# Project-SEA-Stack/HydroChrono

Measured on AMD Instinct MI355X. Metric: hydro-force evals/sec (all bodies), higher is better.
Workload: dtype f64

## Files before the change

hydrochrono_amd/capi.py:

```python
import ctypes as C
import os

_PKG = os.path.dirname(os.path.abspath(__file__))
LIB_PATH = os.path.join(_PKG, "lib", "libhydrochrono_amd.so")
TUNING_LIB_PATH = os.path.join(_PKG, "lib", "libhydrochrono_amd_tuning.so")

HC_OK, HC_ERR_RUNTIME, HC_ERR_OUT_OF_RANGE, HC_ERR_INVALID, HC_ERR_DEVICE, HC_ERR_UNSUPPORTED = range(6)

c_double_p = C.POINTER(C.c_double)
c_int_p = C.POINTER(C.c_int)


class IrregularWaveParams(C.Structure):
    _fields_ = [("num_bodies", C.c_int), ("simulation_dt", C.c_double), ("simulation_duration", C.c_double),
                ("ramp_duration", C.c_double), ("wave_height", C.c_double), ("wave_period", C.c_double),
                ("frequency_min", C.c_double), ("frequency_max", C.c_double), ("nfrequencies", C.c_double),
                ("peak_enhancement_factor", C.c_double), ("is_normalized", C.c_int), ("seed", C.c_int)]


class TaperedDirectOptions(C.Structure):
    _fields_ = [("smoothing", C.c_int), ("window_length", C.c_int), ("rirf_end_time", C.c_double),
                ("taper_start_percent", C.c_double), ("taper_end_percent", C.c_double),
                ("taper_final_amplitude", C.c_double), ("export_plot_csv", C.c_int)]

# ... 15 lines not shown
                ("hydrostatics_calls", C.c_int), ("radiation_calls", C.c_int), ("waves_calls", C.c_int),
                ("conv_kernel_seconds", C.c_double), ("conv_kernel_launches", C.c_longlong),
                ("conv_kernel_bytes", C.c_double), ("block_kernel_seconds", C.c_double),
                ("block_kernel_launches", C.c_longlong), ("block_kernel_bytes", C.c_double),
                ("block_kernel_bytes_once", C.c_double),
                ("step_kernel_seconds", C.c_double), ("step_kernel_launches", C.c_longlong),
                ("scatter_kernel_seconds", C.c_double), ("scatter_kernel_launches", C.c_longlong),
                ("direct_dispatches", C.c_longlong), ("hip_launches", C.c_longlong), ("history_rewinds", C.c_longlong),
                ("mini_pass_seconds", C.c_double), ("mini_pass_launches", C.c_longlong), ("queue_parkings", C.c_longlong),
                ("ahead_pass_slices", C.c_longlong), ("ahead_blocks", C.c_longlong),
                ("pass_lane_launches", C.c_longlong),
                ("multi_doorbell_offset_last", C.c_double), ("multi_doorbell_offset_sum", C.c_double), ("multi_calls", C.c_longlong),
                ("slot_state_steps", C.c_longlong), ("wide_fused_steps", C.c_longlong),
                ("schedule_blocks_ahead", C.c_longlong), ("schedule_blocks_at_start", C.c_longlong), ("ring_grows_for_pass", C.c_longlong),
                ("hot_steps", C.c_longlong), ("tail_launches", C.c_longlong), ("tail_seconds", C.c_double),
                ("tail_bytes", C.c_double), ("tail_blocks", C.c_longlong)]


class InitStats(C.Structure):
    _fields_ = [("h5_read_seconds", C.c_double), ("h5_read_bytes", C.c_double), ("rirf_h2d_seconds", C.c_double), ("rirf_h2d_bytes", C.c_double),
                ("rirf_relayout_seconds", C.c_double), ("rirf_relayout_bytes", C.c_double), ("finalize_seconds", C.c_double),
                ("direct_setup_seconds", C.c_double), ("wave_resample_seconds", C.c_double), ("wave_spectrum_seconds", C.c_double),
                ("wave_eta_seconds", C.c_double), ("wave_eta_samples", C.c_longlong), ("wave_eta_components", C.c_longlong),
                ("wave_eta_mode", C.c_int), ("pad_", C.c_int), ("wave_upload_seconds", C.c_double), ("wave_upload_bytes", C.c_double),
                ("wave_total_seconds", C.c_double), ("taper_seconds", C.c_double), ("taper_bytes", C.c_double),
                ("synth_seconds", C.c_double), ("synth_bytes", C.c_double)]


SIGNATURES = {
    "hc_version": (C.c_char_p, []),
    "hc_device_count": (C.c_int, []),
# ... 179 lines not shown
```

hydrochrono_amd/csrc/hc_context.hpp:

```cpp
#pragma once
#include <hip/hip_runtime.h>

#include <chrono>
#include <deque>
#include <stdexcept>
#include <string>
#include <vector>

#include "../../include/hydrochrono_amd.h"
#include "hc_direct.hpp"
#include "hc_kernels.hpp"
#include "hc_plan.hpp"

namespace hc {

struct Error : std::runtime_error {
    int status;
    Error(int st, const std::string& what) : std::runtime_error(what), status(st) {}
};

#define HC_HIP(expr)                                                                                          \
    do {                                                                                                      \
        hipError_t _e = (expr);                                                                               \
        if (_e != hipSuccess)                                                                                 \
// ... 256 lines not shown
    int mt_mini = 2;
    int mt_narrow = 2;
    int mt_block = 4, mt_block_design = 6;
    int num_cus  = 256;
    int lookahead = 0;
    hc::Plan plan;
    unsigned long long plan_serial = 0;
    int pass_ahead = 0, pass_slices = 8, pe_cur = 0;
    bool ahead_now = false;
    int gap_seen = 0, gap_long = 0, gap_long_lo = 0;
    double gap_threshold = 4e-6;
    double gap_hint = -1.0;
    std::chrono::steady_clock::time_point t_multi_end{};
    bool have_t_multi_end = false;
    hc::AheadPass ahead;
    int radiation_tail = 1;
    struct SpectralTail {
        bool khat_ok = false;
        bool active = false;
        int k = 0, Q = 0;
        int cur = 0;
        unsigned far_cur = 0, far_next = 0;
        unsigned long long serial = 0;
        double t0 = 0.0, dt = 0.0;
    } spec;
    hc::DeviceBuffer<double> d_khat, d_tail_xw, d_tail_yfar, d_tail_out, d_tail_tw;
    hc::DirectKernel dk_tail_fwd, dk_tail_gemv, dk_tail_inv;
    hc::DeviceBuffer<double> d_partials_far;
    hc::DeviceBuffer<double> d_partials_next;
    bool pass_concurrent = true;
    int pass_lane = 0, pass_free_cus = 4;

    hc::DeviceBuffer<double> d_state, d_hs, d_rad, d_waves, d_total;
    hc::DeviceBuffer<double> d_scratch;
    hc::DeviceBuffer<int> d_err;
    hc::PinnedBuffer<double> h_state, h_out, h_am;
    hc::BarBuffer<double> bar_state;
    hc::BarBuffer<double> bar_am;
    hc::PinnedBuffer<unsigned long long> h_tag_am;
    int am_lane = 0;
    hc::BarBuffer<double> bar_selftest;
    hc::PinnedBuffer<unsigned long long> h_tag_selftest;
// ... 31 lines not shown
```

hydrochrono_amd/csrc/hc_internal.hpp:

```cpp
#pragma once
#include <dlfcn.h>
#include <fcntl.h>
#include <unistd.h>
#include <xmmintrin.h>

#include <algorithm>
#include <chrono>
#include <cmath>
#include <cstdint>
#include <cstdio>
#include <cstdlib>
#include <cstring>
#include <fstream>
#include <limits>
#include <memory>
#include <string>
#include <vector>

#include "hc_context.hpp"
#include "hc_history.hpp"
#include "hc_host_math.hpp"

namespace hc {
void eta_synthesis_fft(const std::vector<double>& t, const std::vector<double>& amp, const std::vector<double>& omega,
// ... 108 lines not shown
    hc::Panel kex;
    hc::EtaTable ex;
};
StepViews make_views(const hc_ctx* c);
struct PassSetup {
    hc::BlockArgs b;
    bool exc_block = false;
    double rad_once = 0.0, exc_once = 0.0, bytes_steps = 0.0;
};
PassSetup make_pass(hc_ctx* c, bool with_exc, bool next_block, bool head_only = false);
void issue_pass_chunks(hc_ctx* c, const PassSetup& ps, int first, int last, bool with_items, hipStream_t stream, bool direct, int lane = 0);
void issue_pass_reduce(hc_ctx* c, const PassSetup& ps, double* P, double* E, hipStream_t stream, bool direct, int lane = 0, const double* tail = nullptr,
                       int tail_j0 = 0);
void launch_pass(hc_ctx* c, hipStream_t stream, bool with_exc, bool direct = false, bool spec_goes_on = false);
void spec_drop(hc_ctx* c, bool k_changed);
void spec_build_khat(hc_ctx* c);
void launch_mini_pass(hc_ctx* c, int i0, hipStream_t stream, bool direct, int next_kw = 0, int lane = 0);
void ahead_drop(hc_ctx* c);
void ahead_issue_slice(hc_ctx* c, hipStream_t stream, bool direct);
void ahead_begin(hc_ctx* c, hipStream_t stream, bool with_exc, bool direct);
bool ahead_expected(const hc_ctx* c, unsigned long long ended_serial);
bool ahead_adoptable(const hc_ctx* c, unsigned long long ended_serial);
bool pass_lane_ready(hc_ctx* c);
void pass_lane_drain(hc_ctx* c);

}
}
```

hydrochrono_amd/csrc/hc_kernels.hip:

```cpp
#include "hc_kernels.hpp"

#include <algorithm>
#include <cstdint>
#include <cstdlib>

namespace hc {

static constexpr int kConvThreads = 256;
static constexpr int kWave        = 64;

typedef double dvec2 __attribute__((ext_vector_type(2)));
typedef double dvec2u __attribute__((ext_vector_type(2), aligned(8)));
typedef double dvec4 __attribute__((ext_vector_type(4)));

__host__ __device__ inline size_t panel_offset(int ngp, int row, int f) {
    const int rt = row >> 4, ri = row & 15, gp = f >> 3, j = (f >> 2) & 1, kk = f & 3;
    return ((static_cast<size_t>(rt) * ngp + gp) * 64 + (kk * 16 + ri)) * 2 + j;
}

__global__ void __launch_bounds__(256) relayout_rirf_kernel(const double* __restrict__ Kb, double* __restrict__ K, int ngp, int D, int S,
                                                             int row0, double scale) {
    const size_t F   = (size_t)S * D;
    const size_t gid = (size_t)blockIdx.x * blockDim.x + threadIdx.x;
    if (gid >= 6 * F) return;
// ... 1820 lines not shown
    NearLaunch l;
    a.n_slices = near_slices_for(a.D);
    const int groups = (a.D + 7) / 8 + 1;
    a.gps_per_slice = (((groups + a.n_slices - 1) / a.n_slices) + 3) & ~3;
    l.grid = a.K.ntiles * a.n_slices;
    l.smem = (size_t)max(1, a.n_near) * 8 * a.gps_per_slice * sizeof(double);
    return l;
}

void launch_near_split(const NearArgs& a0, hipStream_t stream) {
    NearArgs a         = a0;
    const NearLaunch l = near_launch_config(a);
    hipLaunchKernelGGL(near_split_kernel, dim3(l.grid), dim3(256), l.smem, stream, a);
}

__global__ void __launch_bounds__(256) scatter_kernel(ScatterArgs a) {
    extern __shared__ __align__(16) unsigned char smem_raw[];
    double* vs = reinterpret_cast<double*>(smem_raw);
    __shared__ double red[4][16];
    const int tid = threadIdx.x, lane = tid & 63, wave = tid >> 6, kk = lane >> 4;
    const int rt = (int)blockIdx.x % a.K.ntiles, rest = (int)blockIdx.x / a.K.ntiles;
    const int si = rest / a.n_slices, sl = rest - si * a.n_slices;
    const int s  = a.s_lo + si;
    const int D  = a.D;
    const int f0 = s * D, f1 = f0 + D;
    const int g0 = (f0 >> 3) + sl * a.gps_per_slice, g1 = min((f1 + 7) >> 3, g0 + a.gps_per_slice);
    const double* __restrict__ kbase = a.K.base + ((size_t)rt * a.K.ngp) * 128 + lane * 2;
    constexpr int PRE = 4;
    dvec2 pre[PRE];
#pragma unroll
    for (int q = 0; q < PRE; ++q) {
        const int gp = g0 + wave + 4 * q;
        pre[q] = gp < g1 ? *reinterpret_cast<const dvec2*>(kbase + (size_t)gp * 128) : dvec2{0.0, 0.0};
    }
    for (int i = tid; i < 8 * a.gps_per_slice; i += 256) {
        const int f = g0 * 8 + i;
// ... 12 lines not shown
    }
#pragma unroll 4
    for (; gp < g1; gp += 4) {
        const dvec2 kv = *reinterpret_cast<const dvec2*>(kbase + (size_t)gp * 128);
        acc = fma(kv.x, u[gp * 8 + kk], acc);
        acc = fma(kv.y, u[gp * 8 + 4 + kk], acc);
    }
    acc += __shfl_xor(acc, 16, kWave);
    acc += __shfl_xor(acc, 32, kWave);
    if (lane < 16) red[wave][lane] = acc;
    __syncthreads();
    if (tid < 16) {
        const double y = (((red[0][tid] + red[1][tid]) + red[2][tid]) + red[3][tid]) * a.width[s];
        for (int t = 0; t < a.n_tgt[si]; ++t) a.Y[(size_t)a.tgt_off[si][t] + (size_t)sl * a.Dpad + rt * 16 + tid] = a.tgt_coef[si][t] * y;
    }
}

ScatterLaunch scatter_launch_config(ScatterArgs& a) {
    ScatterLaunch l;
    a.n_slices = near_slices_for(a.D);
    const int groups = (a.D + 7) / 8 + 1;
    a.gps_per_slice = (((groups + a.n_slices - 1) / a.n_slices) + 3) & ~3;
    l.grid = a.K.ntiles * a.ns * a.n_slices;
    l.smem = (size_t)8 * a.gps_per_slice * sizeof(double);
    return l;
}

void launch_scatter(const ScatterArgs& a0, hipStream_t stream) {
    if (a0.ns <= 0) return;
    ScatterArgs a         = a0;
// ... 208 lines not shown
```

hydrochrono_amd/csrc/hc_kernels.hpp:

```cpp
#pragma once
#include <hip/hip_runtime.h>

#include <cstddef>

#include "hc_limits.hpp"
#include "hc_tail.hpp"

namespace hc {


struct Panel {
    const double* base;
    int ntiles;
    int ngp;
};
inline size_t panel_doubles(int ntiles, int ngp) { return static_cast<size_t>(ntiles) * ngp * 128; }

struct HistoryView {
    const double* state;
    int N, D;
    double t;
    const double* ring_t;
    const double* ring_v;
    const double* ring_vT;
// ... 300 lines not shown
    const double* Yin;
    double* Yout;
    int Dloc, ncols;
    int bin_lo, bin_hi;
    int col_lo, col_hi;
    int x_shift;
    int rows_per_wg;
};

struct TailInvArgs {
    const double* Y;
    const double* tw;
    double* tail;
    int Dloc, Dpad;
};
constexpr int kTailGemvRows = 32;
int tail_gemv_lds_bytes(const TailGemvArgs& g);
int tail_gemv_grid(const TailGemvArgs& g);
void launch_tail_khat(const TailKhatArgs& a, hipStream_t s);
void launch_tail_fwd(const TailFwdArgs& a, hipStream_t s);
void launch_tail_gemv(const TailGemvArgs& a, hipStream_t s);
void launch_tail_inv(const TailInvArgs& a, hipStream_t s);

}
```

hydrochrono_amd/csrc/hc_pass.cpp:

```cpp
#include "hc_internal.hpp"

using namespace hc::detail;

namespace hc {
namespace detail {

StepViews make_views(const hc_ctx* c) {
    StepViews v{};
    const bool irregular = c->wave_kind == hc::kWaveIrregular;
    v.kex.base   = c->d_kex.p;
    v.kex.ntiles = c->ntiles;
    v.kex.ngp    = c->ngp_ex;
    v.ex.L        = c->L;
    v.ex.ex_tau   = c->d_ex_tau.p;
    v.ex.ex_width = c->d_ex_width.p;
    v.ex.eta_t    = c->d_eta_t.p;
    v.ex.eta      = c->d_eta.p;
    v.ex.nt       = c->nt;
    v.ex.eta_dt   = irregular ? (c->eta_record ? c->eta_h : c->irr.simulation_dt) : 1.0;
    v.ex.eta_t0   = (irregular && !c->eta_t.empty()) ? c->eta_t.front() : 0.0;
    return v;
}


// ... 112 lines not shown
    const hc::BlockArgs& b = ps.b;
    hc::ReduceArgs r{b.partials, b.nchunks, b.nchunks_ex, c->Dpad, c->lookahead, P, E, b.item_counter, 0, 0, 0, 0};
    r.tail    = tail;
    r.tail_j0 = tail_j0;
    if (direct) {
        c->dq->dispatch(c->dk_reduce, static_cast<uint32_t>(hc::reduce_block_grid(r)), 256, 0, &r, sizeof r, -1, 0.0, lane);
        c->prof.direct_dispatches += 1;
        return;
    }
    hc::launch_reduce_block(r, stream);
    c->prof.hip_launches += 1;
}

void spec_drop(hc_ctx* c, bool k_changed) {
    c->spec.active = false;
    c->spec.far_cur = c->spec.far_next = 0;
    if (k_changed) c->spec.khat_ok = false;
}

namespace {

bool spec_eligible(const hc_ctx* c, bool direct) {
    const auto& pl = c->plan;
    if (direct && !(c->dk_tail_fwd.ok() && c->dk_tail_gemv.ok() && c->dk_tail_inv.ok())) return false;
    if (c->conv_mode == 1 && !c->proc_ready) return false;
    if (c->pass_ahead == 1 || (c->pass_ahead == 2 && c->ahead_now && pass_ahead_size_ok(c))) return false;
    const int L = c->lookahead;
    const int NP = hc::tail_partitions(c->S);
    if (c->radiation_tail != 1 || (L != 16 && L != 32) || c->D >= 1024 || NP < 1 || NP * c->D > hc::kTailMaxCols) return false;
    if (!pl.valid || pl.own_zero || pl.sub != 0) return false;
    for (int j = 0; j < L; ++j)
        if (pl.s_defer[j] >= 0 || pl.s_cut[j] >= hc::kTailP) return false;
    return hc::tail_grid_ok(c->times, c->tau, pl.dt, pl.tgrid[1]);
}

void spec_twiddles(hc_ctx* c) {
    if (c->d_tail_tw.n >= 2 * hc::kTailN) return;
    std::vector<double> tw(2 * hc::kTailN);
    const double pi = 3.14159265358979323846;
    for (int k = 0; k < hc::kTailN; ++k) {
        const int q = (4 * k) / hc::kTailN, r = k - q * (hc::kTailN / 4);
        const double cr = std::cos(2.0 * pi * r / hc::kTailN), sr = std::sin(2.0 * pi * r / hc::kTailN);
        double co = cr, si = sr;
        if (q == 1) { co = -sr; si = cr; }
// ... 53 lines not shown
    f.tw      = c->d_tail_tw.p;
    f.Xw      = c->d_tail_xw.p;
    c->prof.tail_bytes += 8.0 * NP * D * hc::kTailN + 16.0 * hc::kTailBins * NP * D;
    c->prof.tail_launches += 1;
    if (dd) {
        c->dq->dispatch(c->dk_tail_fwd, static_cast<uint32_t>(NP * D), hc::kTailN / 2, 0, &f, sizeof f, direct_tag(c, hc::kEvTail));
        c->prof.direct_dispatches += 1;
    } else {
        hc::EventPair* ev = ev_begin(c, hc::kEvTail, stream);
        hc::launch_tail_fwd(f, stream);
        ev_end(ev, stream);
        c->prof.hip_launches += 1;
    }
    double* Y = c->d_tail_yfar.p + static_cast<size_t>(sp.cur) * 2 * hc::kTailBins * c->Dloc;
    if (NP > 1) {
        const int nch = hc::tail_far_chunks(sp.Q);
        if (sp.far_cur == 0) {
            spec_dispatch_gemv(c, stream, dd, 0, hc::kTailBins, D, NP * D, hc::tail_x_shift(false, D), nullptr, Y);
        } else {
            for (int k = 0; k < nch; ++k) {
                if (sp.far_cur & (1u << k)) continue;
                int lo, hi;
                hc::tail_chunk_bins(k, nch, &lo, &hi);
                spec_dispatch_gemv(c, stream, dd, lo, hi, D, NP * D, hc::tail_x_shift(false, D), nullptr, Y);
            }
        }
    }
    spec_dispatch_gemv(c, stream, dd, 0, hc::kTailBins, 0, D, 0, NP > 1 ? Y : nullptr, Y);
    hc::TailInvArgs iv{Y, c->d_tail_tw.p, c->d_tail_out.p, c->Dloc, c->Dpad};
    c->prof.tail_bytes += 16.0 * hc::kTailBins * c->Dloc + 8.0 * hc::kTailP * c->Dloc;
    c->prof.tail_launches += 1;
    if (dd) {
        c->dq->dispatch(c->dk_tail_inv, static_cast<uint32_t>(c->Dloc), hc::kTailN / 2, 0, &iv, sizeof iv, direct_tag(c, hc::kEvTail));
        c->prof.direct_dispatches += 1;
    } else {
        hc::EventPair* ev = ev_begin(c, hc::kEvTail, stream);
        hc::launch_tail_inv(iv, stream);
        ev_end(ev, stream);
        c->prof.hip_launches += 1;
    }
// ... 15 lines not shown
            c->d_khat.alloc(nkhat);
            c->spec.khat_ok = false;
        }
    } catch (const Error&) {
        (void)hipGetLastError();
        c->radiation_tail = 0;
        return false;
    }
    spec_twiddles(c);
    if (!c->spec.khat_ok) spec_build_khat(c);
    return c->spec.khat_ok;
}

}

void launch_pass(hc_ctx* c, hipStream_t stream, bool with_exc, bool direct, bool spec_goes_on) {
    auto& sp = c->spec;
    const auto& pl = c->plan;
    const int L = c->lookahead;
    bool use_tail = false;
    if (spec_goes_on && sp.active && sp.k < sp.Q && std::fabs(pl.dt - sp.dt) <= 1e-9 * sp.dt) {
        const double tol = std::max(1e-9 * pl.dt, 64.0 * std::numeric_limits<double>::epsilon() * std::fabs(pl.tgrid[1]));
        use_tail = std::fabs(pl.tgrid[1] - (sp.t0 + sp.k * L * sp.dt)) <= tol;
    }
    bool sb_start = false;
    if (!use_tail) {
        const bool follows = spec_goes_on && sp.active && sp.k == sp.Q &&
                             std::fabs(pl.tgrid[1] - (sp.t0 + sp.k * L * sp.dt)) <=
                                 std::max(1e-9 * pl.dt, 64.0 * std::numeric_limits<double>::epsilon() * std::fabs(pl.tgrid[1])) &&
                             std::fabs(pl.dt - sp.dt) <= 1e-9 * sp.dt;
        const unsigned far_made = follows ? sp.far_next : 0u;
        sp.active = false;
        if (spec_eligible(c, direct) && spec_ready(c)) {
            sp.cur      = follows ? 1 - sp.cur : sp.cur;
            sp.far_cur  = far_made;
            sp.far_next = 0;
            sp.Q        = hc::tail_blocks_per_superblock(L);
            sp.k        = 0;
            sp.t0       = pl.tgrid[1];
            sp.dt       = pl.dt;
            sp.active   = true;
            use_tail = sb_start = true;
        }
    }
    if (!use_tail) {
        const PassSetup ps = make_pass(c, with_exc, false);
        c->plan.has_exc    = ps.exc_block;
        issue_pass_chunks(c, ps, 0, ps.b.nchunks, true, stream, direct);
        issue_pass_reduce(c, ps, rows_P(c, false), rows_E(c, false), stream, direct);
        return;
    }
    if (sb_start) spec_superblock_start(c, stream, direct);
    const PassSetup ps = make_pass(c, with_exc, false, true);
    c->plan.has_exc    = ps.exc_block;
    issue_pass_chunks(c, ps, 0, ps.b.nchunks, true, stream, direct);
    issue_pass_reduce(c, ps, rows_P(c, false), rows_E(c, false), stream, direct, 0, c->d_tail_out.p, sp.k * L);
    const int NP = hc::tail_partitions(c->S);
    if (NP > 1 && sp.k >= 1) {
        const int ch = sp.k - 1, nch = hc::tail_far_chunks(sp.Q);
        int lo, hi;
        hc::tail_chunk_bins(ch, nch, &lo, &hi);
        spec_dispatch_gemv(c, stream, direct, lo, hi, c->D, NP * c->D, hc::tail_x_shift(true, c->D), nullptr,
                           c->d_tail_yfar.p + static_cast<size_t>(1 - sp.cur) * 2 * hc::kTailBins * c->Dloc);
        sp.far_next |= 1u << ch;
    }
    sp.k += 1;
    sp.serial = c->plan_serial;
    c->prof.tail_blocks += 1;
}

void ahead_drop(hc_ctx* c) { c->ahead.active = false; }

void reset_schedule_state(hc_ctx* c) {
    c->gap_seen = c->gap_long = c->gap_long_lo = 0;
    c->gap_hint  = -1.0;
    c->ahead_now = hc::near_slices_for(c->D) > 1 && c->gap_threshold <= 0.0;
}

bool schedule_ahead_for_next_block(hc_ctx* c) {
// ... 237 lines not shown
```

hydrochrono_amd/csrc/hc_runtime.cpp:

```cpp
#include "hc_internal.hpp"

#include <sched.h>

#include <cctype>

#include <atomic>

using namespace hc::detail;

template <class T>
void hc::BarBuffer<T>::alloc(size_t count) {
    if (p) (void)hipFree(p);
    p       = nullptr;
    n       = 0;
    host_ok = false;
    if (count == 0) return;
    static const bool disabled = HC_TUNE_INT("HC_NO_BAR_STATE", 0) != 0;
    if (disabled) return;
    void* q = nullptr;
    if (hipExtMallocWithFlags(&q, count * sizeof(T), hipDeviceMallocFinegrained) != hipSuccess) {
        (void)hipGetLastError();
        return;
    }
    p = static_cast<T*>(q);
// ... 596 lines not shown
    if (c->dk_finalize_slot.kernarg != sizeof(hc::FinalizeArgs) || c->dk_finalize_slot.priv != 0) c->dk_finalize_slot = hc::DirectKernel{};
    c->slot_state = HC_TUNE_INT("HC_SLOT_STATE", 1) != 0 && c->dk_finalize_slot.ok() && c->N <= hc::kSlotStateMaxBodies;
    c->dk_step_hot[0] = q->find("step_hot_kernelILi1EEEv");
    c->dk_step_hot[1] = q->find("step_hot_kernelILi2EEEv");
    for (auto& k : c->dk_step_hot)
        if (k.kernarg != sizeof(hc::StepHotArgs) || k.priv != 0) k = hc::DirectKernel{};
    c->step_hot = c->slot_state && c->dk_step_hot[0].ok() && c->dk_step_hot[1].ok() && HC_TUNE_INT("HC_STEP_HOT", 1) != 0;
    c->step_halves = HC_TUNE_INT("HC_STEP_HALVES", 1) == 2 ? 2 : 1;
    c->dk_reduce   = q->find("reduce_block_kernelE");
    c->dk_tail_fwd  = q->find("tail_fft_fwdENS_11TailFwdArgsE");
    c->dk_tail_gemv = q->find("tail_gemvENS_12TailGemvArgsE");
    c->dk_tail_inv  = q->find("tail_fft_invENS_11TailInvArgsE");
    if (c->dk_tail_fwd.kernarg != sizeof(hc::TailFwdArgs) || c->dk_tail_gemv.kernarg != sizeof(hc::TailGemvArgs) ||
        c->dk_tail_inv.kernarg != sizeof(hc::TailInvArgs) || c->dk_tail_fwd.priv || c->dk_tail_gemv.priv || c->dk_tail_inv.priv)
        c->dk_tail_fwd = c->dk_tail_gemv = c->dk_tail_inv = hc::DirectKernel{};
    c->dk_added_mass = q->find("added_mass_mv_tagged_kernelE");
    {
        hc::StepArgs a{};
        a.ngroups = 1;
        const hc::StepLaunch l = hc::step_launch_config(a, c->mt);
        char frag[64];
        std::snprintf(frag, sizeof frag, "conv_step_kernelILi%dELi%dEEEv", l.MT, hc::StepLaunch::U);
        c->dk_step = q->find(frag);
        if (c->dk_step.kernarg != sizeof(hc::StepArgs) || c->dk_step.priv != 0) c->dk_step = hc::DirectKernel{};
    }
    for (int depth : {16, 32}) {
        hc::BlockArgs a{}, b{};
        a.depth = depth;
        a.ngroups = 1;
        const hc::BlockLaunch l = hc::block_launch_config(a, c->mt_block, &b);
// ... 95 lines not shown
```

hydrochrono_amd/csrc/hc_step.cpp:

```cpp
#include "hc_internal.hpp"
#include "hc_fanout.hpp"

using namespace hc::detail;

namespace hc {
namespace detail {

bool canary_enabled() {
    static const bool on = HC_TUNE_INT("HC_STEP_CANARY", 1) != 0;
    return on;
}

bool wave_window_ok(const hc_ctx* c, double t) {
    if (c->wave_kind != hc::kWaveIrregular || c->eta_t.size() < 2 || c->ex_groups.empty()) return false;
    const double tmin = c->eta_t.front(), tmax = c->eta_t.back();
    for (const auto& g : c->ex_groups) {
        const double q0 = t - g.tau_front, q1 = t - g.tau_back;
        if (!(tmin <= q0 && q0 <= tmax) || !(tmin <= q1 && q1 <= tmax)) return false;
        if (q0 > tmin && q0 < tmax && q0 <= c->eta_t[1]) return false;
    }
    return true;
}

void check_wave_ready(hc_ctx* c, double t) {
// ... 86 lines not shown
    sa.K     = rad_panel(c);
    sa.D     = c->D;
    sa.Dpad  = c->Dpad;
    sa.s_lo  = pl.scat_lo[m];
    sa.ns    = pl.scat_hi[m] - pl.scat_lo[m] + 1;
    sa.v     = c->d_ring_v.p + static_cast<size_t>(c->head) * c->D;
    sa.width = c->d_width.p;
    sa.Y     = c->d_Y.p;
    for (int si = 0; si < sa.ns; ++si) {
        const int s_ = sa.s_lo + si;
        sa.n_tgt[si] = pl.n_tgt[m][s_];
        for (int t = 0; t < pl.n_tgt[m][s_]; ++t) {
            sa.tgt_off[si][t]  = (pl.tgt_step[m][s_][t] * hc::kTermMax + pl.tgt_k[m][s_][t]) * c->Dpad;
            sa.tgt_coef[si][t] = pl.tgt_coef[m][s_][t];
        }
    }
    if (direct) {
        const hc::ScatterLaunch l = hc::scatter_launch_config(sa);
        c->dq->dispatch(c->dk_scatter, static_cast<uint32_t>(l.grid), 256, static_cast<uint32_t>(l.smem), &sa, sizeof sa, direct_tag(c, hc::kEvScatter));
        c->prof.direct_dispatches += 1;
    } else {
        hc::EventPair* ev = ev_begin(c, hc::kEvScatter, bs);
        hc::launch_scatter(sa, bs);
        c->prof.hip_launches += 1;
        ev_end(ev, bs);
    }
}

void enqueue_tail(hc_ctx* c) {
    if (!c->tail.pending) return;
// ... 1101 lines not shown
        float ms = 0.0f;
        HC_HIP(hipEventElapsedTime(&ms, a, b));
        total_ms += ms;
    }
    (void)hipEventDestroy(a);
    (void)hipEventDestroy(b);
    *mean_us = 1e3 * total_ms / std::max(1, reps);
    if (bytes_once) *bytes_once = ps.rad_once;
    c->plan = hc::Plan{};
    HC_API_END(c)
}
#endif

int hc_set_radiation_tail(hc_ctx* c, int mode) {
    HC_API_BEGIN(c)
    require(mode == 0 || mode == 1, HC_ERR_INVALID, "mode must be 0 (full pass) or 1 (spectral tail where eligible)");
    c->radiation_tail = mode;
    c->spec.active    = false;
    HC_API_END(c)
}

int hc_set_pass_schedule(hc_ctx* c, int one_block_ahead, int slices) {
    HC_API_BEGIN(c)
    require(c->finalized, HC_ERR_INVALID, "hc_finalize has not been called");
    HC_HIP(hipDeviceSynchronize());
    c->pass_ahead   = one_block_ahead < 0 ? default_pass_ahead(c) : (one_block_ahead ? 1 : 0);
    reset_schedule_state(c);
    c->pass_slices  = slices > 0 ? std::min(slices, hc::kDepthDefault - 1) : default_pass_slices(c);
    c->ahead.active = false;
    c->spec.active  = false;
    alloc_partials(c);
// ... 211 lines not shown
```

hydrochrono_amd/csrc/hc_tail.hpp:

```cpp
#pragma once
#include <algorithm>
#include <cmath>
#include <deque>
#include <limits>
#include <vector>

namespace hc {

constexpr int kTailP    = 256;
constexpr int kTailN    = 2 * kTailP;
constexpr int kTailBins = kTailP + 1;
constexpr int kTailMaxCols = 4096;

inline int tail_partitions(int S) { return S >= 2 * kTailP ? (S + kTailP - 1) / kTailP - 1 : 0; }

inline int tail_blocks_per_superblock(int lookahead) { return lookahead > 0 ? kTailP / lookahead : 0; }

inline int tail_far_chunks(int Q) { return Q > 1 ? Q - 1 : 1; }
inline void tail_chunk_bins(int k, int nchunks, int* lo, int* hi) {
    *lo = static_cast<int>(static_cast<long long>(k) * kTailBins / nchunks);
    *hi = static_cast<int>(static_cast<long long>(k + 1) * kTailBins / nchunks);
}

inline int tail_window_back(int a, int k) { return (a + 1) * kTailP - 1 - k; }
inline bool tail_window_live(int S, int a, int k) { return k >= 1 && tail_window_back(a, k) <= S - 2; }

inline int tail_col(int p, int col, int D) { return (p - 1) * D + col; }
inline int tail_x_shift(bool next_superblock, int D) { return next_superblock ? -D : 0; }

inline bool tail_grid_ok(const std::deque<double>& times, const std::vector<double>& tau, double dt, double t_first) {
    const int S = static_cast<int>(tau.size());
    if (tail_partitions(S) < 1 || !(dt > 0.0) || static_cast<int>(times.size()) < S) return false;
    const double tol_t = std::max(1e-9 * dt, 64.0 * std::numeric_limits<double>::epsilon() * std::fabs(t_first));
    if (std::fabs(t_first - (times[0] + dt)) > tol_t) return false;
    for (int k = 1; k < S; ++k)
        if (std::fabs(times[static_cast<size_t>(k)] - (times[0] - k * dt)) > tol_t) return false;
    const double tol_s = std::max(1e-9 * dt, 64.0 * std::numeric_limits<double>::epsilon() * std::fabs(tau.back()));
    for (int s = 0; s < S; ++s)
// ... 7 lines not shown
```

hydrochrono_amd/csrc/hc_tail_kernels.hpp:

```cpp
#pragma once

namespace hc {

static constexpr int kTailThreads = 256;

__device__ __forceinline__ void tail_fft_lds(double* __restrict__ re, double* __restrict__ im, const double* __restrict__ tw, bool inverse) {
    const int t = threadIdx.x;
    __syncthreads();
#pragma unroll 1
    for (int len = 2; len <= kTailN; len <<= 1) {
        const int half = len >> 1;
        const int pos  = t & (half - 1);
        const int i    = (t - pos) * 2 + pos;
        const int j    = i + half;
        const int k    = pos * (kTailN / len);
        const double wr = tw[2 * k], wi = inverse ? -tw[2 * k + 1] : tw[2 * k + 1];
        const double br = re[j], bi = im[j];
        const double pr = wr * br - wi * bi, pi = wr * bi + wi * br;
        const double ar = re[i], ai = im[i];
        re[i] = ar + pr;
        im[i] = ai + pi;
        re[j] = ar - pr;
        im[j] = ai - pi;
        __syncthreads();
// ... 49 lines not shown
        im[kr] = 0.0;
    }
    tail_fft_lds(re, im, a.tw, false);
    const size_t ncols = static_cast<size_t>(a.NP) * a.D;
    const size_t c     = static_cast<size_t>(w - 1) * a.D + col;
    for (int b = t; b < kTailBins; b += kTailThreads) {
        double* dst = a.Xw + 2 * (static_cast<size_t>(b) * ncols + c);
        dst[0] = re[b];
        dst[1] = im[b];
    }
}

static constexpr int kTailGemvUnroll = 6;
static constexpr int kTailGemvBatch  = 4;

__global__ void __launch_bounds__(256) tail_gemv(TailGemvArgs a) {
    extern __shared__ double xs[];
    const int nbin_rows = (a.Dloc + a.rows_per_wg - 1) / a.rows_per_wg;
    const int bin       = a.bin_lo + blockIdx.x / nbin_rows;
    const int row0      = (blockIdx.x % nbin_rows) * a.rows_per_wg;
    const int n         = a.col_hi - a.col_lo;
    const double* __restrict__ xsrc = a.Xw + 2 * (static_cast<size_t>(bin) * a.ncols + a.col_lo + a.x_shift);
    for (int i = threadIdx.x; i < 2 * n; i += 256) xs[i] = xsrc[i];
    __syncthreads();
    const int lane = threadIdx.x & 63, wave = threadIdx.x >> 6;
    const int row_end = min(a.Dloc, row0 + a.rows_per_wg);
    const dvec2* __restrict__ kbin = reinterpret_cast<const dvec2*>(a.Khat + 2 * (static_cast<size_t>(bin) * a.Dloc * a.ncols + a.col_lo));
    for (int rb = row0 + wave * kTailGemvBatch; rb < row_end; rb += 4 * kTailGemvBatch) {
        double sr[kTailGemvBatch], si[kTailGemvBatch];
#pragma unroll
        for (int q = 0; q < kTailGemvBatch; ++q) sr[q] = si[q] = 0.0;
        for (int c0 = 0; c0 < n; c0 += 64 * kTailGemvUnroll) {
            dvec2 kv[kTailGemvBatch][kTailGemvUnroll];
#pragma unroll
            for (int q = 0; q < kTailGemvBatch; ++q) {
                const int row = min(rb + q, row_end - 1);
#pragma unroll
                for (int u = 0; u < kTailGemvUnroll; ++u) {
                    const int c = c0 + 64 * u + lane;
                    kv[q][u] = c < n ? __builtin_nontemporal_load(kbin + static_cast<size_t>(row) * a.ncols + c) : dvec2{0.0, 0.0};
                }
            }
#pragma unroll
            for (int u = 0; u < kTailGemvUnroll; ++u) {
                const int c = c0 + 64 * u + lane;
                const double xr = c < n ? xs[2 * c] : 0.0, xi = c < n ? xs[2 * c + 1] : 0.0;
#pragma unroll
                for (int q = 0; q < kTailGemvBatch; ++q) {
                    sr[q] = fma(kv[q][u].x, xr, sr[q]);
                    sr[q] = fma(-kv[q][u].y, xi, sr[q]);
                    si[q] = fma(kv[q][u].x, xi, si[q]);
                    si[q] = fma(kv[q][u].y, xr, si[q]);
                }
            }
        }
#pragma unroll
        for (int off = 32; off >= 1; off >>= 1) {
#pragma unroll
            for (int q = 0; q < kTailGemvBatch; ++q) {
                sr[q] += __shfl_xor(sr[q], off, 64);
                si[q] += __shfl_xor(si[q], off, 64);
            }
        }
        if (lane < kTailGemvBatch && rb + lane < row_end) {
            double yr = sr[0], yi = si[0];
#pragma unroll
            for (int q = 1; q < kTailGemvBatch; ++q)
                if (lane == q) {
                    yr = sr[q];
                    yi = si[q];
                }
            const size_t o = 2 * (static_cast<size_t>(bin) * a.Dloc + rb + lane);
            if (a.Yin) {
                yr = a.Yin[o] + yr;
                yi = a.Yin[o + 1] + yi;
            }
            a.Yout[o]     = yr;
            a.Yout[o + 1] = yi;
        }
    }
}

__global__ void __launch_bounds__(kTailThreads) tail_fft_inv(TailInvArgs a) {
    __shared__ double re[kTailN], im[kTailN];
    const int t   = threadIdx.x;
    const int row = blockIdx.x;
    for (int k = t; k < kTailN; k += kTailThreads) {
        const int b = k <= kTailP ? k : kTailN - k;
        const double* y = a.Y + 2 * (static_cast<size_t>(b) * a.Dloc + row);
        const double yr = y[0];
        double yi       = (b == 0 || b == kTailP) ? 0.0 : y[1];
        if (k > kTailP) yi = -yi;
        const int kr = tail_bitrev(k);
        re[kr] = yr;
        im[kr] = yi;
    }
    tail_fft_lds(re, im, a.tw, true);
    for (int j = t; j < kTailP; j += kTailThreads) a.tail[static_cast<size_t>(j) * a.Dpad + row] = re[kTailP + j] * (1.0 / kTailN);
}

int tail_gemv_lds_bytes(const TailGemvArgs& g) { return 16 * (g.col_hi - g.col_lo); }
int tail_gemv_grid(const TailGemvArgs& g) { return (g.bin_hi - g.bin_lo) * ((g.Dloc + g.rows_per_wg - 1) / g.rows_per_wg); }

void launch_tail_khat(const TailKhatArgs& a, hipStream_t s) {
    hipLaunchKernelGGL(tail_khat_kernel, dim3(static_cast<unsigned>(a.Dloc) * a.NP * a.D), dim3(kTailThreads), 0, s, a);
}
void launch_tail_fwd(const TailFwdArgs& a, hipStream_t s) {
    hipLaunchKernelGGL(tail_fft_fwd, dim3(static_cast<unsigned>(a.NP) * a.D), dim3(kTailThreads), 0, s, a);
}
void launch_tail_gemv(const TailGemvArgs& a, hipStream_t s) {
    hipLaunchKernelGGL(tail_gemv, dim3(static_cast<unsigned>(tail_gemv_grid(a))), dim3(256), static_cast<unsigned>(tail_gemv_lds_bytes(a)), s, a);
}
void launch_tail_inv(const TailInvArgs& a, hipStream_t s) {
    hipLaunchKernelGGL(tail_fft_inv, dim3(static_cast<unsigned>(a.Dloc)), dim3(kTailThreads), 0, s, a);
}

}
```

include/hydrochrono_amd.h:

```cpp
#ifndef HYDROCHRONO_AMD_H
#define HYDROCHRONO_AMD_H

#include <stddef.h>

#ifdef __cplusplus
extern "C" {
#endif

typedef struct hc_ctx hc_ctx;

typedef enum hc_status {
    HC_OK               = 0,
    HC_ERR_RUNTIME      = 1,
    HC_ERR_OUT_OF_RANGE = 2,
    HC_ERR_INVALID      = 3,
    HC_ERR_DEVICE       = 4,
    HC_ERR_UNSUPPORTED  = 5
} hc_status;

const char* hc_version(void);
int hc_device_count(void);
int hc_device_local_cpus(int device_id, char* out, size_t out_bytes);
int hc_bind_thread_to_device(int device_id);
int hc_create(int num_bodies, int device_id, hc_ctx** out);
// ... 113 lines not shown
    long long queue_parkings;
    long long ahead_pass_slices;
    long long ahead_blocks;
    long long pass_lane_launches;
    double multi_doorbell_offset_last, multi_doorbell_offset_sum;
    long long multi_calls;
    long long slot_state_steps;
    long long wide_fused_steps;
    long long schedule_blocks_ahead, schedule_blocks_at_start;
    long long ring_grows_for_pass;
    long long hot_steps;
    long long tail_launches;
    double tail_seconds;
    double tail_bytes;
    long long tail_blocks;
} hc_profile_stats;
int hc_enable_profiling(hc_ctx* ctx, int on);
int hc_get_profile(hc_ctx* ctx, hc_profile_stats* out);
int hc_reset_profile(hc_ctx* ctx);

typedef struct hc_init_stats {
    double h5_read_seconds, h5_read_bytes;
    double rirf_h2d_seconds, rirf_h2d_bytes;
    double rirf_relayout_seconds, rirf_relayout_bytes;
    double finalize_seconds;
    double direct_setup_seconds;
    double wave_resample_seconds;
    double wave_spectrum_seconds;
    double wave_eta_seconds;
    long long wave_eta_samples, wave_eta_components;
// ... 70 lines not shown
```

Baseline: 77260.

## Let far-bin tail GEMV work ride inside scatter kernel launches

Adds a scatter_ride_kernel that appends spectral-tail far-bin GEMV blocks to the scatter grid, so far bins are computed in small slices alongside each step's scatter instead of as separate GEMV launches. A bitmap tracks which bins are done, and a weighted schedule decides how many bins are due at each step. The tail GEMV is also refactored to stage x in fixed-size LDS tiles instead of one dynamic buffer, which adds a sync per tile. The default radiation_tail mode becomes 2, which keeps separate far-chunk launches, so the ride path runs only when mode 1 is chosen.

```diff
diff --git a/hydrochrono_amd/capi.py b/hydrochrono_amd/capi.py
--- a/hydrochrono_amd/capi.py
+++ b/hydrochrono_amd/capi.py
@@ -53,7 +53,8 @@
                 ("slot_state_steps", C.c_longlong), ("wide_fused_steps", C.c_longlong),
                 ("schedule_blocks_ahead", C.c_longlong), ("schedule_blocks_at_start", C.c_longlong), ("ring_grows_for_pass", C.c_longlong),
                 ("hot_steps", C.c_longlong), ("tail_launches", C.c_longlong), ("tail_seconds", C.c_double),
-                ("tail_bytes", C.c_double), ("tail_blocks", C.c_longlong)]
+                ("tail_bytes", C.c_double), ("tail_blocks", C.c_longlong),
+                ("tail_ride_bins", C.c_longlong), ("tail_ride_launches", C.c_longlong), ("tail_completed_bins", C.c_longlong)]
 
 
 class InitStats(C.Structure):
diff --git a/hydrochrono_amd/csrc/hc_context.hpp b/hydrochrono_amd/csrc/hc_context.hpp
--- a/hydrochrono_amd/csrc/hc_context.hpp
+++ b/hydrochrono_amd/csrc/hc_context.hpp
@@ -294,18 +294,18 @@
     std::chrono::steady_clock::time_point t_multi_end{};
     bool have_t_multi_end = false;
     hc::AheadPass ahead;
-    int radiation_tail = 1;
+    int radiation_tail = 2;
     struct SpectralTail {
         bool khat_ok = false;
         bool active = false;
         int k = 0, Q = 0;
         int cur = 0;
-        unsigned far_cur = 0, far_next = 0;
+        hc::TailBinMap far_cur, far_next;
         unsigned long long serial = 0;
         double t0 = 0.0, dt = 0.0;
     } spec;
     hc::DeviceBuffer<double> d_khat, d_tail_xw, d_tail_yfar, d_tail_out, d_tail_tw;
-    hc::DirectKernel dk_tail_fwd, dk_tail_gemv, dk_tail_inv;
+    hc::DirectKernel dk_tail_fwd, dk_tail_gemv, dk_tail_inv, dk_scatter_ride;
     hc::DeviceBuffer<double> d_partials_far;
     hc::DeviceBuffer<double> d_partials_next;
     bool pass_concurrent = true;
diff --git a/hydrochrono_amd/csrc/hc_internal.hpp b/hydrochrono_amd/csrc/hc_internal.hpp
--- a/hydrochrono_amd/csrc/hc_internal.hpp
+++ b/hydrochrono_amd/csrc/hc_internal.hpp
@@ -146,6 +146,8 @@
                        int tail_j0 = 0);
 void launch_pass(hc_ctx* c, hipStream_t stream, bool with_exc, bool direct = false, bool spec_goes_on = false);
 void spec_drop(hc_ctx* c, bool k_changed);
+bool spec_ride_on(const hc_ctx* c, bool direct);
+bool spec_ride_bins(hc_ctx* c, int m, bool direct, hc::TailRideArgs* r);
 void spec_build_khat(hc_ctx* c);
 void launch_mini_pass(hc_ctx* c, int i0, hipStream_t stream, bool direct, int next_kw = 0, int lane = 0);
 void ahead_drop(hc_ctx* c);
diff --git a/hydrochrono_amd/csrc/hc_kernels.hip b/hydrochrono_amd/csrc/hc_kernels.hip
--- a/hydrochrono_amd/csrc/hc_kernels.hip
+++ b/hydrochrono_amd/csrc/hc_kernels.hip
@@ -1858,12 +1858,9 @@
     hipLaunchKernelGGL(near_split_kernel, dim3(l.grid), dim3(256), l.smem, stream, a);
 }
 
-__global__ void __launch_bounds__(256) scatter_kernel(ScatterArgs a) {
-    extern __shared__ __align__(16) unsigned char smem_raw[];
-    double* vs = reinterpret_cast<double*>(smem_raw);
-    __shared__ double red[4][16];
+__device__ __forceinline__ void scatter_body(const ScatterArgs& a, const int block, double* __restrict__ vs, double (*__restrict__ red)[16]) {
     const int tid = threadIdx.x, lane = tid & 63, wave = tid >> 6, kk = lane >> 4;
-    const int rt = (int)blockIdx.x % a.K.ntiles, rest = (int)blockIdx.x / a.K.ntiles;
+    const int rt = block % a.K.ntiles, rest = block / a.K.ntiles;
     const int si = rest / a.n_slices, sl = rest - si * a.n_slices;
     const int s  = a.s_lo + si;
     const int D  = a.D;
@@ -1906,6 +1903,12 @@
         const double y = (((red[0][tid] + red[1][tid]) + red[2][tid]) + red[3][tid]) * a.width[s];
         for (int t = 0; t < a.n_tgt[si]; ++t) a.Y[(size_t)a.tgt_off[si][t] + (size_t)sl * a.Dpad + rt * 16 + tid] = a.tgt_coef[si][t] * y;
     }
+}
+
+__global__ void __launch_bounds__(256) scatter_kernel(ScatterArgs a) {
+    extern __shared__ __align__(16) unsigned char smem_raw[];
+    __shared__ double red[4][16];
+    scatter_body(a, (int)blockIdx.x, reinterpret_cast<double*>(smem_raw), red);
 }
 
 ScatterLaunch scatter_launch_config(ScatterArgs& a) {
diff --git a/hydrochrono_amd/csrc/hc_kernels.hpp b/hydrochrono_amd/csrc/hc_kernels.hpp
--- a/hydrochrono_amd/csrc/hc_kernels.hpp
+++ b/hydrochrono_amd/csrc/hc_kernels.hpp
@@ -338,6 +338,23 @@
     double* tail;
     int Dloc, Dpad;
 };
+struct TailRideArgs {
+    const double* Khat;
+    const double* Xw;
+    double* Yout;
+    int Dloc, ncols;
+    int col_lo, col_hi;
+    int x_shift;
+    int bin_lo, bin_hi;
+};
+struct ScatterRideArgs {
+    ScatterArgs s;
+    TailRideArgs r;
+};
+constexpr int kTailRideRows = 16;
+constexpr int kTailRideMaxBins = 4;
+inline int tail_ride_items(const TailRideArgs& r) { return (r.bin_hi - r.bin_lo) * ((r.Dloc + kTailRideRows - 1) / kTailRideRows); }
+void launch_scatter_ride(const ScatterRideArgs& a, hipStream_t stream);
 constexpr int kTailGemvRows = 32;
 int tail_gemv_lds_bytes(const TailGemvArgs& g);
 int tail_gemv_grid(const TailGemvArgs& g);
diff --git a/hydrochrono_amd/csrc/hc_pass.cpp b/hydrochrono_amd/csrc/hc_pass.cpp
--- a/hydrochrono_amd/csrc/hc_pass.cpp
+++ b/hydrochrono_amd/csrc/hc_pass.cpp
@@ -150,7 +150,8 @@
 
 void spec_drop(hc_ctx* c, bool k_changed) {
     c->spec.active = false;
-    c->spec.far_cur = c->spec.far_next = 0;
+    c->spec.far_cur.clear();
+    c->spec.far_next.clear();
     if (k_changed) c->spec.khat_ok = false;
 }
 
@@ -163,7 +164,7 @@
     if (c->pass_ahead == 1 || (c->pass_ahead == 2 && c->ahead_now && pass_ahead_size_ok(c))) return false;
     const int L = c->lookahead;
     const int NP = hc::tail_partitions(c->S);
-    if (c->radiation_tail != 1 || (L != 16 && L != 32) || c->D >= 1024 || NP < 1 || NP * c->D > hc::kTailMaxCols) return false;
+    if (c->radiation_tail < 1 || (L != 16 && L != 32) || c->D >= 1024 || NP < 1 || NP * c->D > hc::kTailMaxCols) return false;
     if (!pl.valid || pl.own_zero || pl.sub != 0) return false;
     for (int j = 0; j < L; ++j)
         if (pl.s_defer[j] >= 0 || pl.s_cut[j] >= hc::kTailP) return false;
@@ -247,16 +248,10 @@
     }
     double* Y = c->d_tail_yfar.p + static_cast<size_t>(sp.cur) * 2 * hc::kTailBins * c->Dloc;
     if (NP > 1) {
-        const int nch = hc::tail_far_chunks(sp.Q);
-        if (sp.far_cur == 0) {
-            spec_dispatch_gemv(c, stream, dd, 0, hc::kTailBins, D, NP * D, hc::tail_x_shift(false, D), nullptr, Y);
-        } else {
-            for (int k = 0; k < nch; ++k) {
-                if (sp.far_cur & (1u << k)) continue;
-                int lo, hi;
-                hc::tail_chunk_bins(k, nch, &lo, &hi);
-                spec_dispatch_gemv(c, stream, dd, lo, hi, D, NP * D, hc::tail_x_shift(false, D), nullptr, Y);
-            }
+        int lo, hi;
+        for (int from = 0; sp.far_cur.next_missing(from, hc::kTailBins, &lo, &hi); from = hi) {
+            spec_dispatch_gemv(c, stream, dd, lo, hi, D, NP * D, hc::tail_x_shift(false, D), nullptr, Y);
+            c->prof.tail_completed_bins += hi - lo;
         }
     }
     spec_dispatch_gemv(c, stream, dd, 0, hc::kTailBins, 0, D, 0, NP > 1 ? Y : nullptr, Y);
@@ -302,6 +297,32 @@
 
 }
 
+bool spec_ride_on(const hc_ctx* c, bool direct) { return c->radiation_tail == 1 && (!direct || c->dk_scatter_ride.ok()); }
+
+bool spec_ride_bins(hc_ctx* c, int m, bool direct, hc::TailRideArgs* r) {
+    auto& sp = c->spec;
+    const int NP = hc::tail_partitions(c->S);
+    if (!sp.active || sp.serial != c->plan_serial || NP < 2 || sp.k < 1 || !spec_ride_on(c, direct)) return false;
+    const int want = hc::tail_bins_due(sp.k - 1, m, sp.Q, c->lookahead) - sp.far_next.count();
+    int lo, hi;
+    if (want <= 0 || !sp.far_next.next_missing(0, std::min(want, hc::kTailRideCap), &lo, &hi)) return false;
+    r->Khat    = c->d_khat.p;
+    r->Xw      = c->d_tail_xw.p;
+    r->Yout    = c->d_tail_yfar.p + static_cast<size_t>(1 - sp.cur) * 2 * hc::kTailBins * c->Dloc;
+    r->Dloc    = c->Dloc;
+    r->ncols   = NP * c->D;
+    r->col_lo  = c->D;
+    r->col_hi  = NP * c->D;
+    r->x_shift = hc::tail_x_shift(true, c->D);
+    r->bin_lo  = lo;
+    r->bin_hi  = hi;
+    sp.far_next.set(lo, hi);
+    c->prof.tail_ride_bins += hi - lo;
+    c->prof.tail_ride_launches += 1;
+    c->prof.tail_bytes += 16.0 * (hi - lo) * (static_cast<double>(c->Dloc) * (r->col_hi - r->col_lo) + (r->col_hi - r->col_lo) + c->Dloc);
+    return true;
+}
+
 void launch_pass(hc_ctx* c, hipStream_t stream, bool with_exc, bool direct, bool spec_goes_on) {
     auto& sp = c->spec;
     const auto& pl = c->plan;
@@ -317,12 +338,12 @@
                              std::fabs(pl.tgrid[1] - (sp.t0 + sp.k * L * sp.dt)) <=
                                  std::max(1e-9 * pl.dt, 64.0 * std::numeric_limits<double>::epsilon() * std::fabs(pl.tgrid[1])) &&
                              std::fabs(pl.dt - sp.dt) <= 1e-9 * sp.dt;
-        const unsigned far_made = follows ? sp.far_next : 0u;
+        const hc::TailBinMap far_made = follows ? sp.far_next : hc::TailBinMap{};
         sp.active = false;
         if (spec_eligible(c, direct) && spec_ready(c)) {
             sp.cur      = follows ? 1 - sp.cur : sp.cur;
             sp.far_cur  = far_made;
-            sp.far_next = 0;
+            sp.far_next.clear();
             sp.Q        = hc::tail_blocks_per_superblock(L);
             sp.k        = 0;
             sp.t0       = pl.tgrid[1];
@@ -344,13 +365,13 @@
     issue_pass_chunks(c, ps, 0, ps.b.nchunks, true, stream, direct);
     issue_pass_reduce(c, ps, rows_P(c, false), rows_E(c, false), stream, direct, 0, c->d_tail_out.p, sp.k * L);
     const int NP = hc::tail_partitions(c->S);
-    if (NP > 1 && sp.k >= 1) {
+    if (NP > 1 && sp.k >= 1 && !spec_ride_on(c, direct)) {
         const int ch = sp.k - 1, nch = hc::tail_far_chunks(sp.Q);
         int lo, hi;
         hc::tail_chunk_bins(ch, nch, &lo, &hi);
         spec_dispatch_gemv(c, stream, direct, lo, hi, c->D, NP * c->D, hc::tail_x_shift(true, c->D), nullptr,
                            c->d_tail_yfar.p + static_cast<size_t>(1 - sp.cur) * 2 * hc::kTailBins * c->Dloc);
-        sp.far_next |= 1u << ch;
+        sp.far_next.set(lo, hi);
     }
     sp.k += 1;
     sp.serial = c->plan_serial;
diff --git a/hydrochrono_amd/csrc/hc_runtime.cpp b/hydrochrono_amd/csrc/hc_runtime.cpp
--- a/hydrochrono_amd/csrc/hc_runtime.cpp
+++ b/hydrochrono_amd/csrc/hc_runtime.cpp
@@ -634,6 +634,9 @@
     if (c->dk_tail_fwd.kernarg != sizeof(hc::TailFwdArgs) || c->dk_tail_gemv.kernarg != sizeof(hc::TailGemvArgs) ||
         c->dk_tail_inv.kernarg != sizeof(hc::TailInvArgs) || c->dk_tail_fwd.priv || c->dk_tail_gemv.priv || c->dk_tail_inv.priv)
         c->dk_tail_fwd = c->dk_tail_gemv = c->dk_tail_inv = hc::DirectKernel{};
+    c->dk_scatter_ride = q->find("scatter_ride_kernelE");
+    if (c->dk_scatter_ride.kernarg != sizeof(hc::ScatterRideArgs) || c->dk_scatter_ride.priv != 0) c->dk_scatter_ride = hc::DirectKernel{};
+    static_assert(sizeof(hc::ScatterRideArgs) <= hc::DirectQueue::kSlotBytes, "scatter_ride_kernel's argument block does not fit a kernarg slot");
     c->dk_added_mass = q->find("added_mass_mv_tagged_kernelE");
     {
         hc::StepArgs a{};
diff --git a/hydrochrono_amd/csrc/hc_step.cpp b/hydrochrono_amd/csrc/hc_step.cpp
--- a/hydrochrono_amd/csrc/hc_step.cpp
+++ b/hydrochrono_amd/csrc/hc_step.cpp
@@ -124,6 +124,22 @@
             sa.tgt_off[si][t]  = (pl.tgt_step[m][s_][t] * hc::kTermMax + pl.tgt_k[m][s_][t]) * c->Dpad;
             sa.tgt_coef[si][t] = pl.tgt_coef[m][s_][t];
         }
+    }
+    hc::ScatterRideArgs ride{};
+    if (sa.ns > 0 && spec_ride_bins(c, m, direct, &ride.r)) {
+        ride.s = sa;
+        if (direct) {
+            const hc::ScatterLaunch l = hc::scatter_launch_config(ride.s);
+            c->dq->dispatch(c->dk_scatter_ride, static_cast<uint32_t>(l.grid + hc::tail_ride_items(ride.r)), 256, static_cast<uint32_t>(l.smem), &ride, sizeof ride,
+                            direct_tag(c, hc::kEvScatter));
+            c->prof.direct_dispatches += 1;
+        } else {
+            hc::EventPair* ev = ev_begin(c, hc::kEvScatter, bs);
+            hc::launch_scatter_ride(ride, bs);
+            c->prof.hip_launches += 1;
+            ev_end(ev, bs);
+        }
+        return;
     }
     if (direct) {
         const hc::ScatterLaunch l = hc::scatter_launch_config(sa);
@@ -1255,7 +1271,8 @@
 
 int hc_set_radiation_tail(hc_ctx* c, int mode) {
     HC_API_BEGIN(c)
-    require(mode == 0 || mode == 1, HC_ERR_INVALID, "mode must be 0 (full pass) or 1 (spectral tail where eligible)");
+    require(mode >= 0 && mode <= 2, HC_ERR_INVALID,
+            "mode must be 0 (full pass), 1 (spectral tail where eligible, far bins riding in the scatter launches) or 2 (the tail with its far chunks as launches of their own)");
     c->radiation_tail = mode;
     c->spec.active    = false;
     HC_API_END(c)
diff --git a/hydrochrono_amd/csrc/hc_tail.hpp b/hydrochrono_amd/csrc/hc_tail.hpp
--- a/hydrochrono_amd/csrc/hc_tail.hpp
+++ b/hydrochrono_amd/csrc/hc_tail.hpp
@@ -22,6 +22,40 @@
     *hi = static_cast<int>(static_cast<long long>(k + 1) * kTailBins / nchunks);
 }
 
+struct TailBinMap {
+    unsigned long long w[(kTailBins + 63) / 64] = {};
+    void clear() { for (auto& x : w) x = 0; }
+    bool test(int b) const { return (w[b >> 6] >> (b & 63)) & 1ull; }
+    void set(int lo, int hi) { for (int b = lo; b < hi; ++b) w[b >> 6] |= 1ull << (b & 63); }
+    int count() const { int n = 0; for (int b = 0; b < kTailBins; ++b) n += test(b); return n; }
+    bool next_missing(int from, int cap, int* lo, int* hi) const {
+        int b = from;
+        while (b < kTailBins && test(b)) ++b;
+        if (b >= kTailBins) return false;
+        *lo = b;
+        while (b < kTailBins && !test(b) && b - *lo < cap) ++b;
+        *hi = b;
+        return true;
+    }
+};
+
+constexpr int kTailRideCap = 4;
+constexpr int kTailRideLateWeight = 2;
+inline long long tail_ride_weight_upto(int m, int L, int late_weight) {
+    const int h = L / 2;
+    return m < h ? m : (h - 1) + static_cast<long long>(late_weight) * (m - h + 1);
+}
+inline int tail_bins_due(int k, int m, int Q, int L, int late_weight = kTailRideLateWeight) {
+    if (Q < 1 || L < 2 || k < 0) return 0;
+    if (k >= Q) return kTailBins;
+    m = std::max(0, std::min(m, L - 1));
+    const long long per_block = tail_ride_weight_upto(L - 1, L, late_weight);
+    const long long total     = Q * per_block - late_weight;
+    const long long upto      = k * per_block + tail_ride_weight_upto(m, L, late_weight);
+    if (upto >= total) return kTailBins;
+    return static_cast<int>((upto * kTailBins + total - 1) / total);
+}
+
 inline int tail_window_back(int a, int k) { return (a + 1) * kTailP - 1 - k; }
 inline bool tail_window_live(int S, int a, int k) { return k >= 1 && tail_window_back(a, k) <= S - 2; }
 
diff --git a/hydrochrono_amd/csrc/hc_tail_kernels.hpp b/hydrochrono_amd/csrc/hc_tail_kernels.hpp
--- a/hydrochrono_amd/csrc/hc_tail_kernels.hpp
+++ b/hydrochrono_amd/csrc/hc_tail_kernels.hpp
@@ -87,72 +87,107 @@
 static constexpr int kTailGemvUnroll = 6;
 static constexpr int kTailGemvBatch  = 4;
 
+static constexpr int kTailGemvTile = 64 * kTailGemvUnroll;
+
+__device__ __forceinline__ void tail_row_batch(const dvec2* __restrict__ kbin, size_t ncols, const double* __restrict__ xsrc, int n, int rb, int row_end,
+                                               bool live, double* __restrict__ xt, int bin, int Dloc, const double* __restrict__ Yin, double* __restrict__ Yout) {
+    const int lane = threadIdx.x & 63;
+    double sr[kTailGemvBatch], si[kTailGemvBatch];
+#pragma unroll
+    for (int q = 0; q < kTailGemvBatch; ++q) sr[q] = si[q] = 0.0;
+    for (int c0 = 0; c0 < n; c0 += kTailGemvTile) {
+        dvec2 kv[kTailGemvBatch][kTailGemvUnroll];
+#pragma unroll
+        for (int q = 0; q < kTailGemvBatch; ++q) {
+            const int row = min(rb + q, row_end - 1);
+#pragma unroll
+            for (int u = 0; u < kTailGemvUnroll; ++u) {
+                const int c = c0 + 64 * u + lane;
+                kv[q][u] = (live && c < n) ? __builtin_nontemporal_load(kbin + static_cast<size_t>(row) * ncols + c) : dvec2{0.0, 0.0};
+            }
+        }
+        __syncthreads();
+        const int nt = 2 * min(kTailGemvTile, n - c0);
+        for (int i = threadIdx.x; i < nt; i += 256) xt[i] = xsrc[2 * c0 + i];
+        __syncthreads();
+#pragma unroll
+        for (int u = 0; u < kTailGemvUnroll; ++u) {
+            const int ct = 64 * u + lane;
+            const bool in = c0 + ct < n;
+            const double xr = in ? xt[2 * ct] : 0.0, xi = in ? xt[2 * ct + 1] : 0.0;
+#pragma unroll
+            for (int q = 0; q < kTailGemvBatch; ++q) {
+                sr[q] = fma(kv[q][u].x, xr, sr[q]);
+                sr[q] = fma(-kv[q][u].y, xi, sr[q]);
+                si[q] = fma(kv[q][u].x, xi, si[q]);
+                si[q] = fma(kv[q][u].y, xr, si[q]);
+            }
+        }
+    }
+#pragma unroll
+    for (int off = 32; off >= 1; off >>= 1) {
+#pragma unroll
+        for (int q = 0; q < kTailGemvBatch; ++q) {
+            sr[q] += __shfl_xor(sr[q], off, 64);
+            si[q] += __shfl_xor(si[q], off, 64);
+        }
+    }
+    if (lane < kTailGemvBatch && rb + lane < row_end) {
+        double yr = sr[0], yi = si[0];
+#pragma unroll
+        for (int q = 1; q < kTailGemvBatch; ++q)
+            if (lane == q) {
+                yr = sr[q];
+                yi = si[q];
+            }
+        const size_t o = 2 * (static_cast<size_t>(bin) * Dloc + rb + lane);
+        if (Yin) {
+            yr = Yin[o] + yr;
+            yi = Yin[o + 1] + yi;
+        }
+        Yout[o]     = yr;
+        Yout[o + 1] = yi;
+    }
+}
+
 __global__ void __launch_bounds__(256) tail_gemv(TailGemvArgs a) {
-    extern __shared__ double xs[];
+    __shared__ double xt[2 * kTailGemvTile];
     const int nbin_rows = (a.Dloc + a.rows_per_wg - 1) / a.rows_per_wg;
     const int bin       = a.bin_lo + blockIdx.x / nbin_rows;
     const int row0      = (blockIdx.x % nbin_rows) * a.rows_per_wg;
     const int n         = a.col_hi - a.col_lo;
     const double* __restrict__ xsrc = a.Xw + 2 * (static_cast<size_t>(bin) * a.ncols + a.col_lo + a.x_shift);
-    for (int i = threadIdx.x; i < 2 * n; i += 256) xs[i] = xsrc[i];
-    __syncthreads();
-    const int lane = threadIdx.x & 63, wave = threadIdx.x >> 6;
+    const int wave = threadIdx.x >> 6;
     const int row_end = min(a.Dloc, row0 + a.rows_per_wg);
     const dvec2* __restrict__ kbin = reinterpret_cast<const dvec2*>(a.Khat + 2 * (static_cast<size_t>(bin) * a.Dloc * a.ncols + a.col_lo));
-    for (int rb = row0 + wave * kTailGemvBatch; rb < row_end; rb += 4 * kTailGemvBatch) {
-        double sr[kTailGemvBatch], si[kTailGemvBatch];
-#pragma unroll
-        for (int q = 0; q < kTailGemvBatch; ++q) sr[q] = si[q] = 0.0;
-        for (int c0 = 0; c0 < n; c0 += 64 * kTailGemvUnroll) {
-            dvec2 kv[kTailGemvBatch][kTailGemvUnroll];
-#pragma unroll
-            for (int q = 0; q < kTailGemvBatch; ++q) {
-                const int row = min(rb + q, row_end - 1);
-#pragma unroll
-                for (int u = 0; u < kTailGemvUnroll; ++u) {
-                    const int c = c0 + 64 * u + lane;
-                    kv[q][u] = c < n ? __builtin_nontemporal_load(kbin + static_cast<size_t>(row) * a.ncols + c) : dvec2{0.0, 0.0};
-                }
-            }
-#pragma unroll
-            for (int u = 0; u < kTailGemvUnroll; ++u) {
-                const int c = c0 + 64 * u + lane;
-                const double xr = c < n ? xs[2 * c] : 0.0, xi = c < n ? xs[2 * c + 1] : 0.0;
-#pragma unroll
-                for (int q = 0; q < kTailGemvBatch; ++q) {
-                    sr[q] = fma(kv[q][u].x, xr, sr[q]);
-                    sr[q] = fma(-kv[q][u].y, xi, sr[q]);
-                    si[q] = fma(kv[q][u].x, xi, si[q]);
-                    si[q] = fma(kv[q][u].y, xr, si[q]);
-                }
-            }
-        }
-#pragma unroll
-        for (int off = 32; off >= 1; off >>= 1) {
-#pragma unroll
-            for (int q = 0; q < kTailGemvBatch; ++q) {
-                sr[q] += __shfl_xor(sr[q], off, 64);
-                si[q] += __shfl_xor(si[q], off, 64);
-            }
-        }
-        if (lane < kTailGemvBatch && rb + lane < row_end) {
-            double yr = sr[0], yi = si[0];
-#pragma unroll
-            for (int q = 1; q < kTailGemvBatch; ++q)
-                if (lane == q) {
-                    yr = sr[q];
-                    yi = si[q];
-                }
-            const size_t o = 2 * (static_cast<size_t>(bin) * a.Dloc + rb + lane);
-            if (a.Yin) {
-                yr = a.Yin[o] + yr;
-                yi = a.Yin[o + 1] + yi;
-            }
-            a.Yout[o]     = yr;
-            a.Yout[o + 1] = yi;
-        }
-    }
-}
+    for (int r0 = row0; r0 < row_end; r0 += 4 * kTailGemvBatch) {
+        const int rb = r0 + wave * kTailGemvBatch;
+        tail_row_batch(kbin, static_cast<size_t>(a.ncols), xsrc, n, rb, row_end, rb < row_end, xt, bin, a.Dloc, a.Yin, a.Yout);
+    }
+}
+
+__global__ void __launch_bounds__(256) scatter_ride_kernel(ScatterRideArgs a) {
+    extern __shared__ __align__(16) unsigned char smem_raw[];
+    __shared__ double red[4][16];
+    __shared__ double xt[2 * kTailGemvTile];
+    const int nscatter = a.s.K.ntiles * a.s.ns * a.s.n_slices;
+    if ((int)blockIdx.x < nscatter) {
+        scatter_body(a.s, (int)blockIdx.x, reinterpret_cast<double*>(smem_raw), red);
+        return;
+    }
+    const TailRideArgs& r = a.r;
+    const int item   = (int)blockIdx.x - nscatter;
+    const int groups = (r.Dloc + kTailRideRows - 1) / kTailRideRows;
+    const int bin    = r.bin_lo + item / groups;
+    if (bin >= r.bin_hi) return;
+    const int row0    = (item % groups) * kTailRideRows;
+    const int row_end = min(r.Dloc, row0 + kTailRideRows);
+    const int rb      = row0 + (threadIdx.x >> 6) * kTailGemvBatch;
+    const double* __restrict__ xsrc = r.Xw + 2 * (static_cast<size_t>(bin) * r.ncols + r.col_lo + r.x_shift);
+    const dvec2* __restrict__ kbin = reinterpret_cast<const dvec2*>(r.Khat + 2 * (static_cast<size_t>(bin) * r.Dloc * r.ncols + r.col_lo));
+    tail_row_batch(kbin, static_cast<size_t>(r.ncols), xsrc, r.col_hi - r.col_lo, rb, row_end, rb < row_end, xt, bin, r.Dloc, nullptr, r.Yout);
+}
+static_assert(kTailRideRows == 4 * kTailGemvBatch, "a ride item is one row batch per wave");
 
 __global__ void __launch_bounds__(kTailThreads) tail_fft_inv(TailInvArgs a) {
     __shared__ double re[kTailN], im[kTailN];
@@ -172,7 +207,7 @@
     for (int j = t; j < kTailP; j += kTailThreads) a.tail[static_cast<size_t>(j) * a.Dpad + row] = re[kTailP + j] * (1.0 / kTailN);
 }
 
-int tail_gemv_lds_bytes(const TailGemvArgs& g) { return 16 * (g.col_hi - g.col_lo); }
+int tail_gemv_lds_bytes(const TailGemvArgs&) { return 0; }
 int tail_gemv_grid(const TailGemvArgs& g) { return (g.bin_hi - g.bin_lo) * ((g.Dloc + g.rows_per_wg - 1) / g.rows_per_wg); }
 
 void launch_tail_khat(const TailKhatArgs& a, hipStream_t s) {
@@ -184,6 +219,11 @@
 void launch_tail_gemv(const TailGemvArgs& a, hipStream_t s) {
     hipLaunchKernelGGL(tail_gemv, dim3(static_cast<unsigned>(tail_gemv_grid(a))), dim3(256), static_cast<unsigned>(tail_gemv_lds_bytes(a)), s, a);
 }
+void launch_scatter_ride(const ScatterRideArgs& a0, hipStream_t s) {
+    ScatterRideArgs a     = a0;
+    const ScatterLaunch l = scatter_launch_config(a.s);
+    hipLaunchKernelGGL(scatter_ride_kernel, dim3(static_cast<unsigned>(l.grid + tail_ride_items(a.r))), dim3(256), static_cast<unsigned>(l.smem), s, a);
+}
 void launch_tail_inv(const TailInvArgs& a, hipStream_t s) {
     hipLaunchKernelGGL(tail_fft_inv, dim3(static_cast<unsigned>(a.Dloc)), dim3(kTailThreads), 0, s, a);
 }
diff --git a/include/hydrochrono_amd.h b/include/hydrochrono_amd.h
--- a/include/hydrochrono_amd.h
+++ b/include/hydrochrono_amd.h
@@ -151,6 +151,7 @@
     double tail_seconds;
     double tail_bytes;
     long long tail_blocks;
+    long long tail_ride_bins, tail_ride_launches, tail_completed_bins;
 } hc_profile_stats;
 int hc_enable_profiling(hc_ctx* ctx, int on);
 int hc_get_profile(hc_ctx* ctx, hc_profile_stats* out);
```

Result: no change. 76780 (-0.6%).
